# transferia/transferia

Hardware: NVIDIA H100
Metric: ChangeItems/sec on ClickBench-shaped 99-col batches (filter_rows + cast + ClickHouse native block + LZ4 frames) (higher is better)
Workload: dtype u8

## Files before the change

### transferia_b200/csrc/kernels_encode.cuh

```cuda
#pragma once
#include "device_types.cuh"

namespace tfk {

__device__ __forceinline__ uint32_t warp_incl_scan(uint32_t v) {
    const unsigned lane = threadIdx.x & 31;
#pragma unroll
    for (int d = 1; d < 32; d <<= 1) { uint32_t t = __shfl_up_sync(0xffffffffu, v, d); if (lane >= (unsigned)d) v += t; }
    return v;
}
__device__ __forceinline__ uint32_t block_excl_scan(uint32_t v, uint32_t* total, uint32_t* smem33) {
    const unsigned lane = threadIdx.x & 31, warp = threadIdx.x >> 5, nw = (blockDim.x + 31) >> 5;
    uint32_t inc = warp_incl_scan(v);
    if (lane == 31) smem33[warp] = inc;
    __syncthreads();
    if (warp == 0) {
        uint32_t w = lane < nw ? smem33[lane] : 0;
        uint32_t wi = warp_incl_scan(w);
        smem33[lane] = wi - w;
        if (lane == 31) smem33[32] = wi;
    }
    __syncthreads();
    uint32_t res = inc - v + smem33[warp];
    *total = smem33[32];
// ... 333 lines not shown
            s_size[1][threadIdx.x] = (d.nullable && n) ? n : 0;
            s_size[2][threadIdx.x] = n ? ((d.out_kind == OK_STR || d.out_kind == OK_TOSTR) ? a.col_bytes[d.str_slot] : (uint64_t)d.out_w * n) : 0;
        }
        __syncthreads();
        if (threadIdx.x == 0) {
            uint64_t p = s_run; const int m = a.ncols - base < 256 ? a.ncols - base : 256;
            for (int k = 0; k < m; k++) { s_pos[k] = p; p += s_size[0][k] + s_size[1][k] + s_size[2][k]; }
            s_run = p;
        }
        __syncthreads();
        if (c < a.ncols) {
            DCol& d = a.cols[a.out_cols[c]];
            const uint64_t p = s_pos[threadIdx.x];
            d.hdr_off = p; d.null_off = p + s_size[0][threadIdx.x]; d.out_off = d.null_off + s_size[1][threadIdx.x];
            const uint32_t hb = a.col_header_off[c], hn = (uint32_t)s_size[0][threadIdx.x];
            for (uint32_t k = 0; k < hn; k++) a.raw[p + k] = a.col_headers[hb + k];
        }
    }
    __syncthreads();
    if (threadIdx.x == 0) {
        const uint64_t p = s_run;
        a.st->raw_total = p;
        a.st->n_frames = p ? (p + a.frame_bytes - 1) / a.frame_bytes : 1;
        a.st->frame_ticket = 0;
    }
}
#endif

struct ColRegions { uint64_t values, validity, aux, offsets, heap, heap_len; };

__global__ void k_layout_columnar(LayoutArgs a, ColRegions* regions);
#ifdef TF_KERNELS_ENCODE
__global__ void __launch_bounds__(256) k_layout_columnar(LayoutArgs a, ColRegions* regions) {
    __shared__ uint64_t s_sz[5][256];
    __shared__ uint64_t s_pos[256];
    __shared__ uint64_t s_run;
    const uint64_t n = a.st->n_kept;
    if (threadIdx.x == 0) s_run = 0;
    for (int base = 0; base < a.ncols; base += 256) {
        const int k = base + threadIdx.x;
        __syncthreads();
        if (k < a.ncols) {
            const DCol& d = a.cols[a.out_cols[k]];
            const bool var = d.out_kind == OK_STR || d.out_kind == OK_MASK || d.out_kind == OK_TOSTR;
            const bool fresh = d.out_kind == OK_MASK || d.out_kind == OK_TOSTR || d.out_kind == OK_TODT;
            const uint64_t heap = (d.out_kind == OK_STR || d.out_kind == OK_TOSTR) ? a.col_bytes[d.str_slot] : (d.out_kind == OK_MASK ? 64 * n : 0);
            s_sz[0][threadIdx.x] = var ? 0 : (uint64_t)d.out_w * n;
            s_sz[1][threadIdx.x] = (d.validity && !fresh) ? (n + 7) / 8 : 0;
            s_sz[2][threadIdx.x] = (d.aux && !fresh) ? (d.type == TF_ANY ? n : 4 * n) : 0;
            s_sz[3][threadIdx.x] = var ? 4 * (n + 1) : 0;
            s_sz[4][threadIdx.x] = heap;
        }
        __syncthreads();
        if (threadIdx.x == 0) {
            uint64_t p = s_run; const int m = a.ncols - base < 256 ? a.ncols - base : 256;
            for (int q = 0; q < m; q++) { s_pos[q] = p; for (int z = 0; z < 5; z++) p += (s_sz[z][q] + 15) & ~15ull; }
            s_run = p;
        }
        __syncthreads();
        if (k < a.ncols) {
            DCol& d = a.cols[a.out_cols[k]];
            uint64_t p = s_pos[threadIdx.x]; ColRegions r;
            auto take = [&](int z) { const uint64_t at = p; p += (s_sz[z][threadIdx.x] + 15) & ~15ull; return at; };
            const uint64_t v = take(0), val = take(1), ax = take(2), of = take(3), hp = take(4);
            const bool var = d.out_kind == OK_STR || d.out_kind == OK_MASK || d.out_kind == OK_TOSTR;
            d.out_off = var ? hp : v; d.null_off = val; d.aux_off = ax; d.offs_off = of;
            r.values = var ? ~0ull : v; r.validity = s_sz[1][threadIdx.x] ? val : ~0ull; r.aux = s_sz[2][threadIdx.x] ? ax : ~0ull;
            r.offsets = var ? of : ~0ull; r.heap = var ? hp : ~0ull; r.heap_len = s_sz[4][threadIdx.x];
            regions[k] = r;
            if (var) ((uint32_t*)(a.raw + of))[n] = (uint32_t)s_sz[4][threadIdx.x];
        }
    }
    __syncthreads();
    if (threadIdx.x == 0) { a.st->raw_total = s_run; a.st->n_frames = 0; a.st->frame_ticket = 0; }
}
#endif

struct EncodeArgs {
    const DCol* cols;
    const int32_t* slots;
    const uint32_t* sel; const DState* st; uint8_t* raw;
    uint32_t* tile_sum; const uint64_t* tile_base; uint32_t ntiles_cap;
    int columnar;
};

#define TF_SLOT_NULLMAP (1 << 30)
#define TF_SLOT_AUX (1 << 29)
#define TF_SLOT_ZEROMAP (1 << 28)
#define TF_FIX_TILE_WORDS 2048
#define CH_MAX_DATE_SEC 4291747200LL

enum StreamKind { SK_COPY = 0, SK_BOOL, SK_DATE, SK_DATETIME, SK_TS64, SK_NULLMAP, SK_AUX32, SK_AUX8, SK_ZERO, SK_TODT_CH, SK_TODT_SEC };

template <int K, int INW> __device__ __forceinline__ uint64_t elem_t(const DCol& c, const uint32_t* sel, uint64_t j, uint64_t n) {
    if (j >= n) return 0;
    const uint64_t r = sel ? sel[j] : j;
    if (K == SK_ZERO) return 0;
    if (K == SK_TODT_CH || K == SK_TODT_SEC) {
        int64_t s = 0;
        if (row_valid(c, r)) s = c.type == TF_INT32 ? (int64_t)((const int32_t*)c.values)[r] : (int64_t)((const uint32_t*)c.values)[r];
        if (K == SK_TODT_SEC) return (uint64_t)s;
        if (s > CH_MAX_DATE_SEC) s = CH_MAX_DATE_SEC;
        if (s < 0) s = 0;
        return (uint64_t)s;
    }
    if (K == SK_AUX8) return (uint64_t)c.aux[r];
    if (K == SK_AUX32) return (uint64_t)((const uint32_t*)c.aux)[r];
    const bool valid = row_valid(c, r);
    if (K == SK_NULLMAP) return valid ? 0 : 1;
    if (!valid) return 0;
    if (K == SK_COPY) {
        if (INW == 1) return c.values[r];
        if (INW == 2) return ((const uint16_t*)c.values)[r];
        if (INW == 4) return ((const uint32_t*)c.values)[r];
        return ((const uint64_t*)c.values)[r];
    }
    if (K == SK_BOOL) return c.values[r] != 0;
    if (K == SK_DATE || K == SK_DATETIME) {
        int64_t s = ((const int64_t*)c.values)[r];
        const uint32_t ns = c.aux ? ((const uint32_t*)c.aux)[r] : 0;
        if (s > CH_MAX_DATE_SEC || (s == CH_MAX_DATE_SEC && ns > 0)) s = CH_MAX_DATE_SEC;
        if (s < 0) s = 0;
        return K == SK_DATE ? (uint64_t)(s / 86400) : (uint64_t)s;
    }
    const int64_t s = ((const int64_t*)c.values)[r];
    const uint32_t ns = c.aux ? ((const uint32_t*)c.aux)[r] : 0;
    return (uint64_t)(s * 1000000LL + (int64_t)(ns / 1000u));
}

template <int K, int INW, int W> __device__ __forceinline__ uint32_t stream_word_t(const DCol& c, const uint32_t* sel, uint64_t q, uint64_t n) {
    if (W == 1) return (uint32_t)elem_t<K, INW>(c, sel, 4 * q, n) | ((uint32_t)elem_t<K, INW>(c, sel, 4 * q + 1, n) << 8) |
                       ((uint32_t)elem_t<K, INW>(c, sel, 4 * q + 2, n) << 16) | ((uint32_t)elem_t<K, INW>(c, sel, 4 * q + 3, n) << 24);
    if (W == 2) return (uint32_t)(elem_t<K, INW>(c, sel, 2 * q, n) & 0xffff) | ((uint32_t)(elem_t<K, INW>(c, sel, 2 * q + 1, n) & 0xffff) << 16);
    if (W == 4) return (uint32_t)elem_t<K, INW>(c, sel, q, n);
    const uint64_t v = elem_t<K, INW>(c, sel, q >> 1, n); return (uint32_t)(v >> ((q & 1) * 32));
}

template <int K, int INW, int W> __device__ __forceinline__ void encode_stream(const DCol& c, const EncodeArgs& a, uint64_t base, uint64_t n) {
    const uint32_t m = (uint32_t)(base & 3);
    const uint64_t total = n * (uint64_t)W;
    const uint64_t T = (m + total + 3) >> 2;
    uint8_t* dst0 = a.raw + (base - m);
    const unsigned lane = threadIdx.x & 31;
    for (uint64_t t0 = (uint64_t)blockIdx.x * TF_FIX_TILE_WORDS; t0 < T; t0 += (uint64_t)gridDim.x * TF_FIX_TILE_WORDS)
#pragma unroll 2
    for (uint32_t it = 0; it < TF_FIX_TILE_WORDS / 256; it++) {
        const uint64_t t = t0 + it * 256 + threadIdx.x;
        const uint32_t wcur = (t < T) ? stream_word_t<K, INW, W>(c, a.sel, t, n) : 0;
        uint32_t wprev = __shfl_up_sync(0xffffffffu, wcur, 1);
        if (lane == 0) wprev = (m && t > 0 && t <= T) ? stream_word_t<K, INW, W>(c, a.sel, t - 1, n) : 0;
        if (t >= T) continue;
        const uint32_t val = m ? __funnelshift_r(wprev, wcur, 8 * (4 - m)) : wcur;
        const int64_t sb = (int64_t)(4 * t) - (int64_t)m;
        uint8_t* dst = dst0 + 4 * t;
        if (sb >= 0 && (uint64_t)sb + 4 <= total) *(uint32_t*)dst = val;
        else {
#pragma unroll
            for (int b = 0; b < 4; b++) { const int64_t x = sb + b; if (x >= 0 && (uint64_t)x < total) dst[b] = (uint8_t)(val >> (8 * b)); }
        }
    }
}

__global__ void k_encode_fixed(EncodeArgs a);
#ifdef TF_KERNELS_ENCODE
__global__ void __launch_bounds__(256) k_encode_fixed(EncodeArgs a) {
    const int32_t slot = a.slots[blockIdx.y];
    const DCol c = a.cols[slot & ~(TF_SLOT_NULLMAP | TF_SLOT_AUX | TF_SLOT_ZEROMAP)];
    const uint64_t n = a.st->n_kept;
    if (n == 0) return;
    const DCol& cc = c;
    if (slot & TF_SLOT_ZEROMAP) { encode_stream<SK_ZERO, 1, 1>(cc, a, c.null_off, n); return; }
    if (slot & TF_SLOT_NULLMAP) { encode_stream<SK_NULLMAP, 1, 1>(c, a, c.null_off, n); return; }
    if (slot & TF_SLOT_AUX) { if (c.type == TF_ANY) encode_stream<SK_AUX8, 1, 1>(c, a, c.aux_off, n); else encode_stream<SK_AUX32, 4, 4>(c, a, c.aux_off, n); return; }
    switch (c.out_kind) {
    case OK_COPY:
        switch (c.in_w) {
        case 1: encode_stream<SK_COPY, 1, 1>(c, a, c.out_off, n); break;
        case 2: encode_stream<SK_COPY, 2, 2>(c, a, c.out_off, n); break;
        case 4: encode_stream<SK_COPY, 4, 4>(c, a, c.out_off, n); break;
        default: encode_stream<SK_COPY, 8, 8>(c, a, c.out_off, n); break;
        }
        break;
    case OK_BOOL: encode_stream<SK_BOOL, 1, 1>(c, a, c.out_off, n); break;
    case OK_DATE: encode_stream<SK_DATE, 8, 2>(c, a, c.out_off, n); break;
    case OK_DATETIME: encode_stream<SK_DATETIME, 8, 4>(c, a, c.out_off, n); break;
    case OK_TS64: encode_stream<SK_TS64, 8, 8>(c, a, c.out_off, n); break;
    case OK_TODT: if (a.columnar) encode_stream<SK_TODT_SEC, 4, 8>(c, a, c.out_off, n); else encode_stream<SK_TODT_CH, 4, 4>(c, a, c.out_off, n); break;
    }
}
#endif

__global__ void k_pack_validity(EncodeArgs a);
#ifdef TF_KERNELS_ENCODE
__global__ void __launch_bounds__(256) k_pack_validity(EncodeArgs a) {
    const DCol c = a.cols[a.slots[blockIdx.y]];
    const uint64_t n = a.st->n_kept;
    const uint64_t b = (uint64_t)blockIdx.x * blockDim.x + threadIdx.x;
    if (b * 8 >= n) return;
    uint32_t v = 0;
#pragma unroll
    for (int k = 0; k < 8; k++) {
        const uint64_t j = b * 8 + k;
        if (j < n) { const uint64_t r = a.sel ? a.sel[j] : j; v |= (row_valid(c, r) ? 1u : 0u) << k; }
    }
    a.raw[c.null_off + b] = (uint8_t)v;
}
#endif


struct MeasureArgs { const DCol* cols; int ncols; uint64_t nrows; uint64_t* per_row; unsigned long long* total; };

__global__ void k_measure(MeasureArgs a);
#ifdef TF_KERNELS_ENCODE
__global__ void __launch_bounds__(256) k_measure(MeasureArgs a) {
    __shared__ uint32_t sm[33];
    const uint64_t r = (uint64_t)blockIdx.x * blockDim.x + threadIdx.x;
    uint64_t sz = 0;
    if (r < a.nrows) {
        sz = 24;
        for (int c = 0; c < a.ncols; c++) {
            const DCol& d = a.cols[c];
            sz += 16;
            if (!row_valid(d, r)) continue;
            switch (d.type) {
            case TF_UTF8: sz += 16 + (d.offsets[r + 1] - d.offsets[r]); break;
            case TF_ANY: sz += 16 + (d.offsets[r + 1] - d.offsets[r]); break;
            case TF_BYTES: sz += 24 + (d.offsets[r + 1] - d.offsets[r]); break;
            case TF_DATE: case TF_DATETIME: case TF_TIMESTAMP: sz += 24; break;
            default: sz += (uint64_t)d.in_w;
            }
        }
        if (a.per_row) a.per_row[r] = sz;
    }
    const uint32_t lo = (uint32_t)(sz & 0xffffffu), hi = (uint32_t)(sz >> 24);
    uint32_t tl, th; block_excl_scan(lo, &tl, sm); __syncthreads(); block_excl_scan(hi, &th, sm);
    if (threadIdx.x == 0) atomicAdd(a.total, (unsigned long long)tl + ((unsigned long long)th << 24));
}
#endif

}
```

### transferia_b200/csrc/tfgpu.cu

```cuda
#include <cuda_runtime.h>
#include <algorithm>
#include <chrono>
#include <cstdio>
#include <cstdlib>
#include <cstring>
#include <memory>
#include <string>
#include <vector>

#include "../../include/tfgpu.h"
#include "../../include/tfgpu_sink.h"
#include "plan.hpp"
#include "device_types.cuh"
#include "launch.hpp"
#include "host_internal.hpp"

using namespace tfk;

namespace {

#define CK(x) do { cudaError_t _e = (x); if (_e != cudaSuccess) throw CudaError{_e, #x}; } while (0)

inline size_t align_up(size_t v, size_t a) { return (v + a - 1) / a * a; }

// ... 203 lines not shown
    }
    pd.n_fsteps = (int)fsteps.size(); pd.n_fixed_slots = (int)pd.fixed_slots.size(); pd.n_str = (int)pd.str_slots.size(); pd.n_mask_cols = (int)pd.mask_slot_cols.size();
    pd.n_tostr = 0; for (size_t c = 0; c < pd.col_out_kind.size(); c++) if (pd.col_out_kind[c] == OK_TOSTR) pd.n_tostr++;
    std::vector<ShardCol> shcols;
    for (size_t k = 0; k < pl.shard_cols.size(); k++) shcols.push_back(ShardCol{pl.shard_cols[k], pl.shard_form[k], 0, 0});
    const std::vector<int32_t> oc(pl.out_cols.begin(), pl.out_cols.end());
    ConstImage ci;
    const size_t o_terms = ci.add(terms.data(), terms.size() * sizeof(DTerm)), o_expr_off = ci.add(expr_off.data(), expr_off.size() * 4),
                 o_fsteps = ci.add(fsteps.data(), fsteps.size() * sizeof(DFilterStep)), o_blob = ci.add(pl.blob.data(), pl.blob.size()),
                 o_hdr = ci.add(pl.col_headers.data(), pl.col_headers.size()), o_hdr_off = ci.add(pl.col_header_off.data(), pl.col_header_off.size() * 4),
                 o_fixed = ci.add(pd.fixed_slots.data(), pd.fixed_slots.size() * 4), o_str = ci.add(pd.str_slots.data(), pd.str_slots.size() * 4),
                 o_mask = ci.add(pd.mask_slot_cols.data(), pd.mask_slot_cols.size() * 4), o_keys = ci.add(keys.data(), keys.size() * sizeof(MaskKey)),
                 o_out = ci.add(oc.data(), oc.size() * 4), o_jcols = ci.add(jcols.data(), jcols.size() * sizeof(JsonCol)), o_jnames = ci.add(jnames.data(), jnames.size()),
                 o_sjcols = ci.add(sjcols.data(), sjcols.size() * sizeof(JsonCol)), o_scsv = ci.add(scsvcols.data(), scsvcols.size() * sizeof(JsonCol)),
                 o_snames = ci.add(snames.data(), snames.size()), o_shard = ci.add(shcols.data(), shcols.size() * sizeof(ShardCol));
    uint8_t* P = ci.upload(pd.consts);
    pd.d_terms = (DTerm*)(P + o_terms); pd.d_expr_off = (uint32_t*)(P + o_expr_off); pd.d_fsteps = (DFilterStep*)(P + o_fsteps); pd.d_blob = P + o_blob;
    pd.d_col_headers = P + o_hdr; pd.d_col_header_off = (uint32_t*)(P + o_hdr_off);
    pd.d_fixed_slots = (int32_t*)(P + o_fixed); pd.d_str_slots = (int32_t*)(P + o_str); pd.d_mask_slots = (int32_t*)(P + o_mask); pd.d_mask_keys = (MaskKey*)(P + o_keys);
    pd.d_out_cols = (int32_t*)(P + o_out); pd.d_jcols = (JsonCol*)(P + o_jcols); pd.d_jnames = P + o_jnames;
    pd.d_sjcols = (JsonCol*)(P + o_sjcols); pd.d_scsvcols = (JsonCol*)(P + o_scsv); pd.d_snames = P + o_snames; pd.d_shard_cols = (ShardCol*)(P + o_shard);
}

struct Sizes { uint64_t raw_bound, n_frames_max, wire_bound; uint32_t ntiles_cap, nblocks; };

Sizes compute_sizes(const tfgpu_engine* e, const PlanDev& pd, uint64_t n, const tf_col* cols, bool columnar, bool json) {
    const tfplan::Plan& pl = pd.plan;
    uint64_t raw = 64 + pl.col_headers.size();
    for (int oc : pl.out_cols) {
        const size_t c = (size_t)oc;
        if (pd.col_nullable[c]) raw += n;
        bool n2f = false; for (int q : pl.n2f_cols) if ((size_t)q == c) n2f = true;
        if (pd.col_out_kind[c] == OK_STR) raw += (n2f ? 6 : 1) * cols[c].heap_len + 5 * n;
        else if (pd.col_out_kind[c] == OK_TOSTR) raw += (in_width(cols[c].type) ? 40 * n : (n2f ? 36 : 6) * cols[c].heap_len + 8 * n) + 5 * n;
        else raw += (uint64_t)pd.col_out_w[c] * n;
        if (columnar) raw += 8 * n + 4 * (n + 1) + n / 8 + 6 * 16 + (pd.col_out_kind[c] == OK_MASK ? 64 * n : 0);
        if (json) raw += (uint64_t)(pl.in_schema[c].name.size() + 4 + 48) * n + (in_width(cols[c].type) ? 0 : (n2f ? 36 : 6) * cols[c].heap_len);
    }
    Sizes s;
    s.raw_bound = raw + 256;
    s.n_frames_max = (raw + e->frame_bytes - 1) / e->frame_bytes + 1;
    s.wire_bound = s.n_frames_max * (uint64_t)(LZ_HDR + lz4_bound(e->frame_bytes)) + 1024;
    s.ntiles_cap = (uint32_t)((n + TF_STR_TILE - 1) / TF_STR_TILE + 1);
    s.nblocks = (uint32_t)((n + 255) / 256 + 1);
    return s;
}


static void launch_offsets(tfgpu_engine* e, const uint32_t* d_len, uint64_t nrows, uint32_t nslots, uint32_t* d_off, uint64_t* d_tot, cudaStream_t s) {
    const uint32_t nchunks = (uint32_t)((nrows + CSV_OFF_CHUNK - 1) / CSV_OFF_CHUNK);
    if (!nchunks || !nslots) { TF_LAUNCH(e, k_csv_offsets, nslots ? nslots : 1, 1024, 0, s, d_len, nrows, d_off, d_tot); return; }
    e->off_scratch.ensure((size_t)nslots * nchunks * 8 + 256);
    uint64_t* cs = (uint64_t*)e->off_scratch.p;
    TF_LAUNCH(e, k_offsets_sum, dim3(nchunks, nslots), 1024, 0, s, d_len, nrows, nchunks, cs);
    TF_LAUNCH(e, k_offsets_chunks, nslots, 32, 0, s, cs, nchunks, d_tot);
    TF_LAUNCH(e, k_offsets_write, dim3(nchunks, nslots), 1024, 0, s, d_len, nrows, nchunks, cs, d_tot, d_off);
}

struct Heaps { std::vector<uint64_t> total, base; };
Heaps size_heaps(tfgpu_engine* e, const uint32_t* d_len, uint64_t nrows, uint32_t k, uint32_t* d_off, uint64_t* d_tot, uint64_t* d_base,
                 DevBuf& heap, const char* too_big) {
    cudaStream_t s = e->stream;
    launch_offsets(e, d_len, nrows, k, d_off, d_tot, s);
    Heaps h{std::vector<uint64_t>(k), std::vector<uint64_t>(k)};
    CK(cudaMemcpyAsync(h.total.data(), d_tot, (size_t)k * 8, cudaMemcpyDeviceToHost, s)); CK(cudaStreamSynchronize(s));
    uint64_t run = 0; for (uint32_t i = 0; i < k; i++) { h.base[i] = run; run += align_up(h.total[i], 16); }
    if (run >= (1ull << 32)) throw tfplan::FatalError(TF_E_FATAL_ARG, too_big);
    heap.ensure(run + 256);
    CK(cudaMemcpyAsync(d_base, h.base.data(), (size_t)k * 8, cudaMemcpyHostToDevice, s));
    return h;
}

DCol make_dcol(const tf_col& ic, int type) {
    DCol d; std::memset(&d, 0, sizeof d);
    d.type = type; d.in_w = in_width(type); d.str_slot = -1; d.mask_slot = -1;
    d.values = (const uint8_t*)ic.values; d.validity = ic.validity; d.offsets = ic.offsets; d.heap = ic.heap; d.aux = (const uint8_t*)ic.aux;
    return d;
}

void ensure_d_cols(tfgpu_engine* e, size_t nc) {
    if (e->d_cols_cap >= nc) return;
    if (e->d_cols) CK(cudaFree(e->d_cols));
    CK(cudaMalloc(&e->d_cols, sizeof(DCol) * nc)); e->d_cols_cap = nc;
}

uint32_t grid_cap(const tfgpu_engine* e, uint32_t tiles_upper, uint32_t nslots, uint32_t waves) {
    const uint32_t want = ((uint32_t)e->sm_count * 6u * waves + nslots - 1) / (nslots ? nslots : 1);
    return std::max(1u, std::min(tiles_upper, std::max(want, 8u)));
}

void run_deflate(tfgpu_engine* e, const uint8_t* text, uint64_t total, bool zlib) {
    cudaStream_t s = e->stream;
    const uint64_t nch = (total + DF_CHUNK - 1) / DF_CHUNK;
    if (nch >= (1ull << 32)) throw tfplan::FatalError(TF_E_FATAL_ARG, "row text too large to compress in one call");
    e->wire.ensure(total + nch * DF_CHUNK_OVERHEAD + 64);
    Layout L;
    const size_t o_pfx = L.take(nch * 8), o_sums = L.take(nch * 8), o_ticket = L.take(4);
    e->defl_meta.ensure(L.total());
    uint8_t* M = e->defl_meta.p;
    CK(cudaMemsetAsync(M + o_pfx, 0, nch * 8, s)); CK(cudaMemsetAsync(M + o_ticket, 0, 4, s));
    DeflateArgs da{text, total, e->wire.p, (unsigned long long*)(M + o_pfx), (uint32_t*)(M + o_sums), (uint32_t*)(M + o_ticket), (uint32_t)nch, zlib ? 1 : 0, e->d_state};
    if (nch) {
        const uint32_t grid = (uint32_t)std::min<uint64_t>(nch, (uint64_t)e->sm_count * 2);
        TF_LAUNCH(e, k_deflate_chunks, grid, DF_THREADS, df_smem().total, s, da);
    }
    TF_LAUNCH(e, k_deflate_finish, 1, 1024, 0, s, da);
}

struct ChainOut { uint8_t* errcode; uint16_t* errstep; const uint32_t* sel; bool has_sharder; };

ChainOut run_chain(tfgpu_engine* e, PlanDev& pd, uint64_t n, const tf_col* dev_cols, const uint8_t* dev_kinds, int out_fmt, const uint8_t* pre_err = nullptr, const DbzEmitArgs* dz = nullptr) {
    const bool columnar = out_fmt == 0;
    const tfplan::Plan& pl = pd.plan;
    const size_t nc = pl.in_schema.size();
    const int wire_base = out_fmt & 0xff;
    const bool dbz = wire_base == TF_WIRE_DEBEZIUM;
    const bool ser = wire_base == TF_WIRE_SER_JSON || wire_base == TF_WIRE_SER_CSV || dbz;
    const bool json_rows = wire_base == TF_WIRE_CH_JSONEACHROW || ser;
    if (ser) for (size_t c = 0; c < nc; c++) if (pd.col_out_kind[c] == OK_TOSTR && pl.in_schema[c].tf == TF_ANY)
        throw tfplan::FatalError(TF_E_FATAL_UNSUPPORTED, "serializer sinks after convert_to_string on an `any` column are not handled on the device");
    const Sizes sz = compute_sizes(e, pd, n, dev_cols, columnar, json_rows);
    cudaStream_t s = e->stream;
    if (e->tail_pending && !(out_fmt == TF_WIRE_CH_NATIVE_LZ4 && n == e->tail_nrows && (const void*)&pd == e->tail_plan && sz.n_frames_max == e->tail_nframes_max)) join_tail(e);
    const size_t nslot_alloc = (size_t)(pd.n_str > 0 ? pd.n_str : 1);
    Layout W;
    const size_t o_keep = W.take(n), o_errcode = W.take(n), o_errstep = W.take(2 * n), o_blockcnt = W.take(sz.nblocks * 4), o_blockoff = W.take(sz.nblocks * 4),
                 o_sel = W.take(n * 4), o_tile_sum = W.take(nslot_alloc * sz.ntiles_cap * 4), o_tile_base = W.take(nslot_alloc * sz.ntiles_cap * 8),
                 o_comp = W.take(sz.n_frames_max * 4), o_wire_off = W.take(sz.n_frames_max * 8), o_pfx = W.take(sz.n_frames_max * 8), o_col_bytes = W.take(nslot_alloc * 8);
    e->work.ensure(W.total());
    uint8_t* w = e->work.p;
    uint8_t* keep = w + o_keep; uint8_t* errcode = w + o_errcode; uint16_t* errstep = (uint16_t*)(w + o_errstep); uint32_t* blockcnt = (uint32_t*)(w + o_blockcnt); uint32_t* blockoff = (uint32_t*)(w + o_blockoff);
    uint32_t* tile_sum = (uint32_t*)(w + o_tile_sum); uint64_t* tile_base = (uint64_t*)(w + o_tile_base); uint64_t* col_bytes = (uint64_t*)(w + o_col_bytes);
    uint32_t* comp_size = (uint32_t*)(w + o_comp); uint64_t* wire_off = (uint64_t*)(w + o_wire_off); unsigned long long* frame_pfx = (unsigned long long*)(w + o_pfx);
    e->raw.ensure(sz.raw_bound);
    const bool lz = out_fmt == TF_WIRE_CH_NATIVE_LZ4;
    if (lz) e->wire.ensure(sz.wire_bound);
    ensure_d_cols(e, nc);
    std::vector<DCol> hc(nc); std::vector<StrictCol> strict;
    for (size_t c = 0; c < nc; c++) {
        const tf_col& ic = dev_cols[c];
        int ctype = ic.type;
        if (ic.type != pl.in_schema[c].tf) {
            const int st = ic.type, dt = pl.in_schema[c].tf;
            const bool s_num = in_width(st) && st != TF_INTERVAL && st != TF_DATE && st != TF_DATETIME && st != TF_TIMESTAMP;
            if ((st == TF_UTF8 && dt == TF_BYTES) || (st == TF_BYTES && dt == TF_UTF8)) ctype = dt;
            else if (s_num && in_width(dt) && !(st == TF_FLOAT && dt == TF_DOUBLE) && !(st == TF_BOOLEAN && dt == TF_DOUBLE)) { strict.push_back(StrictCol{(const uint8_t*)ic.values, nullptr, ic.validity, st, dt, (int32_t)c, 0}); ctype = dt; }
            else throw tfplan::FatalError(TF_E_FATAL_ARG, "column " + std::to_string(c) + ": a " + std::to_string(st) + " value cannot be strictified to the plan's column type on the device");
        }
        DCol& d = hc[c]; d = make_dcol(ic, ctype);
        d.out_kind = pd.col_out_kind[c]; d.out_w = pd.col_out_w[c];
        if (columnar && d.out_kind == OK_TODT) d.out_w = 8;
        else if (columnar && d.out_kind != OK_STR && d.out_kind != OK_MASK && d.out_kind != OK_TOSTR) { d.out_kind = OK_COPY; d.out_w = d.in_w; }
        d.nullable = pd.col_nullable[c]; d.str_slot = pd.col_str_slot[c]; d.mask_slot = pd.col_mask_slot[c];
        if (n) {
            if (d.in_w && !d.values) throw tfplan::FatalError(TF_E_FATAL_ARG, "column " + std::to_string(c) + ": values pointer is NULL");
            if (!d.in_w && !d.offsets) throw tfplan::FatalError(TF_E_FATAL_ARG, "column " + std::to_string(c) + ": offsets pointer is NULL");
        }
    }
    const uint16_t* pre_term = nullptr;
    if (!strict.empty() && n) {
        Layout S;
        const size_t o_desc = S.take(strict.size() * sizeof(StrictCol)), o_err = S.take(n), o_term = S.take(2 * n);
        std::vector<size_t> o_val(strict.size());
        for (size_t k = 0; k < strict.size(); k++) o_val[k] = S.take((size_t)in_width(strict[k].dst_tf) * n + 16);
        e->strict_stage.ensure(S.total() + 256);
        uint8_t* B = e->strict_stage.p;
        for (size_t k = 0; k < strict.size(); k++) { strict[k].dst = B + o_val[k]; hc[strict[k].col].values = B + o_val[k]; }
        CK(cudaMemcpyAsync(B + o_desc, strict.data(), strict.size() * sizeof(StrictCol), cudaMemcpyHostToDevice, s));
        if (pre_err) CK(cudaMemcpyAsync(B + o_err, pre_err, n, cudaMemcpyDeviceToDevice, s)); else CK(cudaMemsetAsync(B + o_err, 0, n, s));
        StrictArgs sa{(const StrictCol*)(B + o_desc), (int)strict.size(), n, B + o_err, (uint16_t*)(B + o_term)};
        TF_LAUNCH(e, k_strictify, (uint32_t)((n + 255) / 256), 256, 0, s, sa);
        pre_err = B + o_err; pre_term = (const uint16_t*)(B + o_term);
    }
    CK(cudaMemcpyAsync(e->d_cols, hc.data(), sizeof(DCol) * nc, cudaMemcpyHostToDevice, s));
    CK(cudaMemsetAsync(e->d_state, 0, sizeof(DState), s));
    if (!pl.n2f_cols.empty() && n) {
        const size_t k2 = pl.n2f_cols.size();
        Layout S;
        const size_t o_which = S.take(k2 * 4), o_len = S.take(k2 * n * 4), o_off = S.take(k2 * (n + 1) * 4), o_tot = S.take(k2 * 8 + 8), o_base = S.take(k2 * 8 + 8), o_err = S.take(n);
        e->n2f_stage.ensure(S.total() + 256);
        uint8_t* B = e->n2f_stage.p;
        std::vector<int32_t> which(pl.n2f_cols.begin(), pl.n2f_cols.end());
        CK(cudaMemcpyAsync(B + o_which, which.data(), k2 * 4, cudaMemcpyHostToDevice, s));
        if (pre_err) CK(cudaMemcpyAsync(B + o_err, pre_err, n, cudaMemcpyDeviceToDevice, s)); else CK(cudaMemsetAsync(B + o_err, 0, n, s));
        N2fArgs na{e->d_cols, (const int32_t*)(B + o_which), dev_kinds, n, (uint32_t*)(B + o_len), (const uint32_t*)(B + o_off), nullptr, (const uint64_t*)(B + o_base), B + o_err};
        TF_LAUNCH(e, k_n2f_sizes, dim3((uint32_t)((n + 127) / 128), (uint32_t)k2), 128, 0, s, na);
        const Heaps h = size_heaps(e, (const uint32_t*)(B + o_len), n, (uint32_t)k2, (uint32_t*)(B + o_off), (uint64_t*)(B + o_tot), (uint64_t*)(B + o_base),
                                   e->n2f_heap, "number_to_float: a rewritten column exceeds 4 GiB");
        na.heap = e->n2f_heap.p;
        TF_LAUNCH(e, k_n2f_write, dim3((uint32_t)((n + 127) / 128), (uint32_t)k2), 128, 0, s, na);
        for (size_t k = 0; k < k2; k++) { DCol& d = hc[pl.n2f_cols[k]]; d.offsets = (const uint32_t*)(B + o_off) + k * (n + 1); d.heap = e->n2f_heap.p + h.base[k]; }
        CK(cudaMemcpyAsync(e->d_cols, hc.data(), sizeof(DCol) * nc, cudaMemcpyHostToDevice, s));
        pre_err = B + o_err;
    }
    const bool sink_guard = dev_kinds && !columnar && !dbz;
    const bool has_filter = pd.n_fsteps > 0 || pre_err || sink_guard;
    e->last_wire_fmt = out_fmt;
    const uint32_t nb = (uint32_t)((n + 255) / 256);
    uint32_t* sel = (has_filter && n) ? (uint32_t*)(w + o_sel) : nullptr;
    if (sel) {
        FilterArgs fa{e->d_cols, dev_kinds, n, pd.d_fsteps, pd.n_fsteps, pd.d_expr_off, pd.d_terms, pd.d_blob, keep, errcode, errstep, blockcnt, e->d_state, pre_err, pre_term, sink_guard ? 1 : 0};
        TF_LAUNCH(e, k_filter, nb, 256, 0, s, fa);
        TF_LAUNCH(e, k_scan_blockcnt, 1, 1024, 0, s, blockcnt, blockoff, nb, e->d_state);
        TF_LAUNCH(e, k_compact_sel, nb, 256, 0, s, keep, blockoff, n, sel);
    }
    const uint32_t ntiles = (uint32_t)((n + TF_STR_TILE - 1) / TF_STR_TILE);
    const uint32_t str_gx = std::max(1u, (ntiles + TF_STR_GROUP - 1) / TF_STR_GROUP);
    EncodeArgs ea{e->d_cols, pd.d_str_slots, sel, e->d_state, e->raw.p, tile_sum, tile_base, sz.ntiles_cap, columnar ? 1 : 0};
    if (!has_filter || !n) {
        DState init; std::memset(&init, 0, sizeof init); init.n_kept = n;
        CK(cudaMemcpyAsync(e->d_state, &init, sizeof init, cudaMemcpyHostToDevice, s));
    }
    if (pl.has_sharder && n) {
        e->part_ids.ensure(n * 4 + 256);
        ShardArgs sa{e->d_cols, pd.d_shard_cols, (int)pl.shard_cols.size(), pd.d_mask_keys, sel, e->d_state, pl.shards, (uint32_t*)e->part_ids.p};
        TF_LAUNCH(e, k_shard_ids, nb, 256, 0, s, sa);
    }
    if (json_rows) {
        const uint32_t jt = (uint32_t)((n + TF_JSON_TILE - 1) / TF_JSON_TILE);
        JsonArgs ja{e->d_cols, ser ? (wire_base == TF_WIRE_SER_CSV ? pd.d_scsvcols : pd.d_sjcols) : pd.d_jcols, (int)pl.out_cols.size(), ser ? pd.d_snames : pd.d_jnames, pd.d_mask_keys, sel, e->d_state, e->raw.p,
                    (uint32_t*)e->work_json_sizes(n), tile_sum, tile_base, col_bytes,
                    dbz ? 3 : ser ? (wire_base == TF_WIRE_SER_JSON ? 1 : 2) : 0, (uint32_t)(((out_fmt & TF_WIRE_F_CLOSING_NEWLINE) ? TF_SER_NL : 0) | ((out_fmt & TF_WIRE_F_ANY_AS_STRING) ? TF_SER_AAS : 0)), errcode, errstep, DbzEmitArgs{}};
        if (dbz) { ja.jcols = pd.d_sjcols; e->dbz_keysz.ensure(n * 4 + 256); e->dbz_msgsz.ensure(n * 28 + 256); ja.dz = *dz; ja.dz.key_size = (uint32_t*)e->dbz_keysz.p; ja.dz.msg_size = (uint32_t*)e->dbz_msgsz.p; }
        if (ser && !has_filter && n) { CK(cudaMemsetAsync(errcode, 0, n, s)); CK(cudaMemsetAsync(errstep, 0, 2 * n, s)); }
        if (jt) TF_LAUNCH(e, k_json_sizes, jt, TF_JSON_TILE, 0, s, ja);
        LayoutArgs lj{e->d_cols, 0, pd.d_out_cols, pd.d_str_slots, 1, tile_sum, tile_base, sz.ntiles_cap, pd.d_col_headers, pd.d_col_header_off,
                      e->raw.p, e->d_state, n, 1, e->frame_bytes, col_bytes};
        TF_LAUNCH(e, k_layout_scan, 1, 1024, 0, s, lj);
        uint64_t json_total = 0;
        {
            CK(cudaMemcpyAsync(&json_total, col_bytes, 8, cudaMemcpyDeviceToHost, s)); CK(cudaStreamSynchronize(s));
            e->raw.ensure(json_total + 256); ja.raw = e->raw.p;
        }
        TF_LAUNCH(e, k_json_write, jt ? jt : 1, TF_JSON_TILE, 0, s, ja);
        if (ser && (out_fmt & (TF_WIRE_F_GZIP | TF_WIRE_F_ZLIB))) run_deflate(e, e->raw.p, n ? json_total : 0, (out_fmt & TF_WIRE_F_ZLIB) != 0);
        return ChainOut{errcode, errstep, sel, pl.has_sharder};
    }
    if (pd.n_str && ntiles) TF_LAUNCH(e, k_str_sizes, dim3(str_gx, pd.n_str), TF_STR_THREADS, 0, s, ea);
    LayoutArgs la{e->d_cols, (int)pl.out_cols.size(), pd.d_out_cols, pd.d_str_slots, pd.n_str, tile_sum, tile_base, sz.ntiles_cap, pd.d_col_headers, pd.d_col_header_off,
                  e->raw.p, e->d_state, n, 1, e->frame_bytes, col_bytes};
    if (pd.n_str) TF_LAUNCH(e, k_layout_scan, pd.n_str, 1024, 0, s, la);
    const int32_t* fixed_slots = pd.d_fixed_slots; uint32_t n_fixed = (uint32_t)pd.n_fixed_slots, n_valid = 0;
    if (!columnar) TF_LAUNCH(e, k_layout_finish, 1, 256, 0, s, la);
    else {
        const size_t no = pl.out_cols.size();
        if (e->d_call_cap < no) {
            if (e->d_call_slots) { CK(cudaFree(e->d_call_slots)); CK(cudaFree(e->d_regions)); }
            CK(cudaMalloc(&e->d_call_slots, sizeof(int32_t) * 3 * no)); CK(cudaMalloc(&e->d_regions, sizeof(ColRegions) * no)); e->d_call_cap = no;
        }
        std::vector<int32_t> fixed, valid;
        for (int oc : pl.out_cols) {
            const DCol& d = hc[oc];
            if (d.out_kind == OK_COPY || d.out_kind == OK_TODT) fixed.push_back(oc);
            const bool fresh = d.out_kind == OK_MASK || d.out_kind == OK_TOSTR || d.out_kind == OK_TODT;
            if (!fresh && d.aux) fixed.push_back(oc | TF_SLOT_AUX);
            if (!fresh && d.validity) valid.push_back(oc);
        }
        fixed_slots = e->d_call_slots; n_fixed = (uint32_t)fixed.size(); n_valid = (uint32_t)valid.size();
        fixed.insert(fixed.end(), valid.begin(), valid.end());
        if (!fixed.empty()) CK(cudaMemcpyAsync(e->d_call_slots, fixed.data(), fixed.size() * 4, cudaMemcpyHostToDevice, s));
        TF_LAUNCH(e, k_layout_columnar, 1, 256, 0, s, la, e->d_regions);
    }
    if (n) {
        if (n_fixed) {
            const uint32_t gx = grid_cap(e, (uint32_t)((2 * n + 2 + TF_FIX_TILE_WORDS - 1) / TF_FIX_TILE_WORDS), n_fixed, 6);
            EncodeArgs fa = ea; fa.slots = fixed_slots;
            TF_LAUNCH(e, k_encode_fixed, dim3(gx, n_fixed), 256, 0, s, fa);
        }
        if (n_valid) {
            EncodeArgs va = ea; va.slots = fixed_slots + n_fixed;
            TF_LAUNCH(e, k_pack_validity, dim3((uint32_t)((n / 8 + 256) / 256), n_valid), 256, 0, s, va);
        }
        if (pd.n_str) TF_LAUNCH(e, k_encode_str_plain, dim3(str_gx, pd.n_str), TF_STR_THREADS, 0, s, ea);
        if (pd.n_str && pd.n_tostr) TF_LAUNCH(e, k_encode_str, dim3(ntiles, pd.n_str), TF_STR_THREADS, 0, s, ea);
        if (pd.n_mask_cols) {
            MaskArgs ma{e->d_cols, pd.d_mask_slots, pd.d_mask_keys, sel, e->d_state, e->raw.p, columnar ? 1 : 0};
            TF_LAUNCH(e, k_mask_encode, dim3((uint32_t)((n + 127) / 128), pd.n_mask_cols), 128, 0, s, ma);
        }
    }
    if (lz) {
        Lz4Args za{e->raw.p, e->d_state, e->wire.p, comp_size, wire_off, frame_pfx, e->d_tail, e->frame_bytes, e->lz_phases};
        const size_t smem = lz_smem(e->frame_bytes).total;
        const uint32_t per_sm = (uint32_t)std::max<size_t>(1, std::min<size_t>(LZ_CTAS_PER_SM, (227 * 1024) / (smem + 1024)));
        const uint32_t grid = (uint32_t)std::min<uint64_t>(sz.n_frames_max, (uint64_t)e->sm_count * per_sm);
        join_tail(e);
        CK(cudaMemsetAsync(frame_pfx, 0, sz.n_frames_max * 8, s));
        TF_LAUNCH(e, k_lz4_frames, grid, LZ_THREADS, smem, s, za);
        FrameArgs fa{comp_size, wire_off, e->wire.p, e->d_tail};
        cudaStream_t s3 = e->side_stream;
        CK(cudaEventRecord(e->ev_fork, s)); CK(cudaStreamWaitEvent(s3, e->ev_fork, 0));
        TF_LAUNCH(e, k_frame_seal, (uint32_t)((sz.n_frames_max + 31) / 32), 32, SEAL_SMEM, s3, fa);
        CK(cudaEventRecord(e->ev_tail, s3));
        e->tail_pending = true; e->tail_nrows = n; e->tail_plan = (const void*)&pd; e->tail_nframes_max = sz.n_frames_max;
    }
    return ChainOut{errcode, errstep, sel, pl.has_sharder};
}

}


static bool wire_is_ser(int wire_fmt) {
    const int b = wire_fmt & 0xff;
    return (b == TF_WIRE_SER_JSON || b == TF_WIRE_SER_CSV) && (wire_fmt & ~(0xff | TF_WIRE_F_CLOSING_NEWLINE | TF_WIRE_F_ANY_AS_STRING | TF_WIRE_F_GZIP | TF_WIRE_F_ZLIB)) == 0 &&
           (wire_fmt & (TF_WIRE_F_GZIP | TF_WIRE_F_ZLIB)) != (TF_WIRE_F_GZIP | TF_WIRE_F_ZLIB);
}
static bool wire_known(int wire_fmt) { return wire_fmt == TF_WIRE_CH_NATIVE || wire_fmt == TF_WIRE_CH_NATIVE_LZ4 || wire_fmt == TF_WIRE_CH_JSONEACHROW || wire_is_ser(wire_fmt); }

static int check_batch(tfgpu_engine* e, int plan_id, const tf_batch* in, PlanDev*& pd) {
    if (!e || !in || plan_id < 0 || plan_id >= (int)e->plans.size()) return TF_E_FATAL_ARG;
    pd = e->plans[plan_id].get();
    if (in->ncols != pd->plan.in_schema.size()) return fail(e, TF_E_FATAL_ARG, "batch column count does not match the plan schema");
    if (in->nrows >= (1ull << 31)) return fail(e, TF_E_FATAL_ARG, "batch too large (>= 2^31 rows)");
    return TF_OK;
}

extern "C" {

const char* tfgpu_version(void) { return "tfgpu 0.1.0 sm_90a"; }

int tfgpu_engine_create(const char* cfg_json, const int* device_ids, int n_devices, tfgpu_engine** out) {
    if (!out) return TF_E_FATAL_ARG;
    *out = nullptr;
    int ndev = 0;
    if (cudaGetDeviceCount(&ndev) != cudaSuccess || ndev == 0) { cudaGetLastError(); return TF_E_FATAL_NODEVICE; }
    if (n_devices > 1) return TF_E_FATAL_ARG;
    auto e = std::make_unique<tfgpu_engine>();
    e->device = (n_devices == 1 && device_ids) ? device_ids[0] : 0;
    if (e->device < 0 || e->device >= ndev) return TF_E_FATAL_ARG;
    try {
        if (cfg_json && *cfg_json) {
            auto cfg = tfj::parse(cfg_json);
            double fb = cfg->get_num("frame_bytes", LZ_MAX_FRAME);
            if (fb < 1024 || fb > LZ_MAX_FRAME || ((uint32_t)fb & 15)) return TF_E_FATAL_CONFIG;
            e->frame_bytes = (uint32_t)fb;
        }
        CK(cudaSetDevice(e->device));
        cudaDeviceProp prop; CK(cudaGetDeviceProperties(&prop, e->device));
        e->sm_count = prop.multiProcessorCount;
        CK(cudaStreamCreateWithFlags(&e->own_stream, cudaStreamNonBlocking));
        e->stream = e->own_stream;
        CK(cudaStreamCreateWithFlags(&e->side_stream, cudaStreamNonBlocking));
        CK(cudaEventCreateWithFlags(&e->ev_tail, cudaEventDisableTiming));
        CK(cudaMalloc(&e->d_tail, 64)); CK(cudaMemset(e->d_tail, 0, 64));
        CK(cudaEventCreateWithFlags(&e->ev_fork, cudaEventDisableTiming));
        CK(cudaMalloc(&e->d_state, sizeof(DState)));
        const struct { const void* k; size_t smem; } big_smem[] = {
            {(const void*)k_lz4_frames, lz_smem(LZ_MAX_FRAME).total}, {(const void*)k_frame_seal, SEAL_SMEM},
            {(const void*)k_dbz_pass1, DBZ_STAGE}, {(const void*)k_deflate_chunks, df_smem().total}};
        for (const auto& b : big_smem) CK(cudaFuncSetAttribute(b.k, cudaFuncAttributeMaxDynamicSharedMemorySize, (int)b.smem));
    } catch (const CudaError& c) { return c.e == cudaErrorMemoryAllocation ? TF_E_RETRY_OOM : TF_E_RETRY_LAUNCH; }
// ... 1036 lines not shown
```

Before: 1.147 billion.

## Rewrite fixed-width column encode as source-row tiles with shared-memory compaction

Replaces the output-word gather encoder, which read each kept row through the sel index, with a source-row-tiled kernel. Each thread loads 8 consecutive input rows with vector loads, compacts the kept rows into shared memory using the keep flags, per-256-row block offsets and a warp scan, then the block writes the output region with aligned 16-byte stores via funnel shifts. The aim is to turn scattered gathers and unaligned byte handling into coalesced reads and wide writes. In exchange it uses 16KB of shared memory per CTA, adds two syncthreads per tile, fixes launch bounds at 6 CTAs, and reads all rows, including filtered ones.

```diff
diff --git a/transferia_b200/csrc/kernels_encode.cuh b/transferia_b200/csrc/kernels_encode.cuh
--- a/transferia_b200/csrc/kernels_encode.cuh
+++ b/transferia_b200/csrc/kernels_encode.cuh
@@ -439,110 +439,157 @@
     const uint32_t* sel; const DState* st; uint8_t* raw;
     uint32_t* tile_sum; const uint64_t* tile_base; uint32_t ntiles_cap;
     int columnar;
+    const uint8_t* keep; const uint32_t* blockoff; uint64_t nrows;
 };
 
 #define TF_SLOT_NULLMAP (1 << 30)
 #define TF_SLOT_AUX (1 << 29)
 #define TF_SLOT_ZEROMAP (1 << 28)
-#define TF_FIX_TILE_WORDS 2048
+#define TF_FIX_ROWS 8
+#define TF_FIX_TILE (256 * TF_FIX_ROWS)
+#define TF_FIX_TILES_PER_CTA 4
 #define CH_MAX_DATE_SEC 4291747200LL
 
 enum StreamKind { SK_COPY = 0, SK_BOOL, SK_DATE, SK_DATETIME, SK_TS64, SK_NULLMAP, SK_AUX32, SK_AUX8, SK_ZERO, SK_TODT_CH, SK_TODT_SEC };
 
-template <int K, int INW> __device__ __forceinline__ uint64_t elem_t(const DCol& c, const uint32_t* sel, uint64_t j, uint64_t n) {
-    if (j >= n) return 0;
-    const uint64_t r = sel ? sel[j] : j;
+template <int K> __device__ __forceinline__ uint64_t cast_elem(const DCol& c, uint64_t v, uint64_t ns, bool valid) {
     if (K == SK_ZERO) return 0;
     if (K == SK_TODT_CH || K == SK_TODT_SEC) {
         int64_t s = 0;
-        if (row_valid(c, r)) s = c.type == TF_INT32 ? (int64_t)((const int32_t*)c.values)[r] : (int64_t)((const uint32_t*)c.values)[r];
+        if (valid) s = c.type == TF_INT32 ? (int64_t)(int32_t)(uint32_t)v : (int64_t)(uint32_t)v;
         if (K == SK_TODT_SEC) return (uint64_t)s;
         if (s > CH_MAX_DATE_SEC) s = CH_MAX_DATE_SEC;
         if (s < 0) s = 0;
         return (uint64_t)s;
     }
-    if (K == SK_AUX8) return (uint64_t)c.aux[r];
-    if (K == SK_AUX32) return (uint64_t)((const uint32_t*)c.aux)[r];
-    const bool valid = row_valid(c, r);
+    if (K == SK_AUX8 || K == SK_AUX32) return v;
     if (K == SK_NULLMAP) return valid ? 0 : 1;
     if (!valid) return 0;
-    if (K == SK_COPY) {
-        if (INW == 1) return c.values[r];
-        if (INW == 2) return ((const uint16_t*)c.values)[r];
-        if (INW == 4) return ((const uint32_t*)c.values)[r];
-        return ((const uint64_t*)c.values)[r];
-    }
-    if (K == SK_BOOL) return c.values[r] != 0;
+    if (K == SK_COPY) return v;
+    if (K == SK_BOOL) return v != 0;
     if (K == SK_DATE || K == SK_DATETIME) {
-        int64_t s = ((const int64_t*)c.values)[r];
-        const uint32_t ns = c.aux ? ((const uint32_t*)c.aux)[r] : 0;
+        int64_t s = (int64_t)v;
         if (s > CH_MAX_DATE_SEC || (s == CH_MAX_DATE_SEC && ns > 0)) s = CH_MAX_DATE_SEC;
         if (s < 0) s = 0;
         return K == SK_DATE ? (uint64_t)(s / 86400) : (uint64_t)s;
     }
-    const int64_t s = ((const int64_t*)c.values)[r];
-    const uint32_t ns = c.aux ? ((const uint32_t*)c.aux)[r] : 0;
-    return (uint64_t)(s * 1000000LL + (int64_t)(ns / 1000u));
-}
-
-template <int K, int INW, int W> __device__ __forceinline__ uint32_t stream_word_t(const DCol& c, const uint32_t* sel, uint64_t q, uint64_t n) {
-    if (W == 1) return (uint32_t)elem_t<K, INW>(c, sel, 4 * q, n) | ((uint32_t)elem_t<K, INW>(c, sel, 4 * q + 1, n) << 8) |
-                       ((uint32_t)elem_t<K, INW>(c, sel, 4 * q + 2, n) << 16) | ((uint32_t)elem_t<K, INW>(c, sel, 4 * q + 3, n) << 24);
-    if (W == 2) return (uint32_t)(elem_t<K, INW>(c, sel, 2 * q, n) & 0xffff) | ((uint32_t)(elem_t<K, INW>(c, sel, 2 * q + 1, n) & 0xffff) << 16);
-    if (W == 4) return (uint32_t)elem_t<K, INW>(c, sel, q, n);
-    const uint64_t v = elem_t<K, INW>(c, sel, q >> 1, n); return (uint32_t)(v >> ((q & 1) * 32));
-}
-
-template <int K, int INW, int W> __device__ __forceinline__ void encode_stream(const DCol& c, const EncodeArgs& a, uint64_t base, uint64_t n) {
-    const uint32_t m = (uint32_t)(base & 3);
-    const uint64_t total = n * (uint64_t)W;
-    const uint64_t T = (m + total + 3) >> 2;
-    uint8_t* dst0 = a.raw + (base - m);
-    const unsigned lane = threadIdx.x & 31;
-    for (uint64_t t0 = (uint64_t)blockIdx.x * TF_FIX_TILE_WORDS; t0 < T; t0 += (uint64_t)gridDim.x * TF_FIX_TILE_WORDS)
-#pragma unroll 2
-    for (uint32_t it = 0; it < TF_FIX_TILE_WORDS / 256; it++) {
-        const uint64_t t = t0 + it * 256 + threadIdx.x;
-        const uint32_t wcur = (t < T) ? stream_word_t<K, INW, W>(c, a.sel, t, n) : 0;
-        uint32_t wprev = __shfl_up_sync(0xffffffffu, wcur, 1);
-        if (lane == 0) wprev = (m && t > 0 && t <= T) ? stream_word_t<K, INW, W>(c, a.sel, t - 1, n) : 0;
-        if (t >= T) continue;
-        const uint32_t val = m ? __funnelshift_r(wprev, wcur, 8 * (4 - m)) : wcur;
-        const int64_t sb = (int64_t)(4 * t) - (int64_t)m;
-        uint8_t* dst = dst0 + 4 * t;
-        if (sb >= 0 && (uint64_t)sb + 4 <= total) *(uint32_t*)dst = val;
-        else {
-#pragma unroll
-            for (int b = 0; b < 4; b++) { const int64_t x = sb + b; if (x >= 0 && (uint64_t)x < total) dst[b] = (uint8_t)(val >> (8 * b)); }
-        }
+    return (uint64_t)((int64_t)v * 1000000LL + (int64_t)(ns / 1000u));
+}
+
+template <int B> __device__ __forceinline__ void load_rows(const uint8_t* p, uint64_t r0, int nr, uint64_t (&v)[TF_FIX_ROWS]) {
+    const uint8_t* q = p + r0 * B;
+    if (nr == TF_FIX_ROWS && ((uintptr_t)q & (B == 1 ? 7 : 15)) == 0) {
+        if (B == 1) {
+            const uint64_t x = *(const uint64_t*)q;
+#pragma unroll
+            for (int k = 0; k < 8; k++) v[k] = (x >> (8 * k)) & 0xff;
+        } else {
+            uint32_t w[2 * B];
+#pragma unroll
+            for (int i = 0; i < B / 2; i++) { const uint4 x = ((const uint4*)q)[i]; w[4 * i] = x.x; w[4 * i + 1] = x.y; w[4 * i + 2] = x.z; w[4 * i + 3] = x.w; }
+#pragma unroll
+            for (int k = 0; k < 8; k++) {
+                if (B == 2) v[k] = (w[k >> 1] >> (16 * (k & 1))) & 0xffff;
+                else if (B == 4) v[k] = w[k];
+                else v[k] = (uint64_t)w[2 * k] | ((uint64_t)w[2 * k + 1] << 32);
+            }
+        }
+        return;
+    }
+#pragma unroll
+    for (int k = 0; k < 8; k++) {
+        const uint64_t r = r0 + k;
+        v[k] = k >= nr ? 0 : B == 1 ? p[r] : B == 2 ? ((const uint16_t*)p)[r] : B == 4 ? ((const uint32_t*)p)[r] : ((const uint64_t*)p)[r];
+    }
+}
+
+__device__ __forceinline__ uint4 bytes_at(const uint4 a, const uint4 b, uint32_t d) {
+    uint32_t x0 = a.x, x1 = a.y, x2 = a.z, x3 = a.w, x4 = b.x, x5 = b.y;
+    if (d & 8) { x0 = x2; x1 = x3; x2 = x4; x3 = x5; x4 = b.z; x5 = b.w; }
+    if (d & 4) { x0 = x1; x1 = x2; x2 = x3; x3 = x4; x4 = x5; }
+    const uint32_t sh = 8 * (d & 3);
+    return make_uint4(__funnelshift_r(x0, x1, sh), __funnelshift_r(x1, x2, sh), __funnelshift_r(x2, x3, sh), __funnelshift_r(x3, x4, sh));
+}
+
+template <int K, int INW, int W> __device__ __forceinline__ void encode_tile(const DCol& c, const EncodeArgs& a, uint64_t base, uint8_t* stage) {
+    constexpr bool VALUES = K != SK_ZERO && K != SK_NULLMAP;
+    constexpr bool VALIDITY = K != SK_ZERO && K != SK_AUX8 && K != SK_AUX32;
+    constexpr bool NANOS = K == SK_DATE || K == SK_DATETIME || K == SK_TS64;
+    const unsigned warp = threadIdx.x >> 5;
+    const uint64_t n = a.nrows, ntiles = (n + TF_FIX_TILE - 1) / TF_FIX_TILE;
+    for (uint64_t tile = blockIdx.x; tile < ntiles; tile += gridDim.x) {
+        const uint64_t t0 = tile * TF_FIX_TILE, r0 = t0 + (uint64_t)threadIdx.x * TF_FIX_ROWS;
+        const int nr = r0 < n ? (int)min((uint64_t)TF_FIX_ROWS, n - r0) : 0;
+        const uint32_t b0 = (uint32_t)(t0 / 256), nb = (uint32_t)((n + 255) / 256);
+        uint64_t kf = 0, j0, j1, bbase;
+        if (a.keep) {
+            if (nr == TF_FIX_ROWS) kf = *(const uint64_t*)(a.keep + r0);
+            else for (int k = 0; k < nr; k++) kf |= (uint64_t)a.keep[r0 + k] << (8 * k);
+            j0 = a.blockoff[b0];
+            j1 = b0 + 8 < nb ? a.blockoff[b0 + 8] : a.st->n_kept;
+            bbase = b0 + warp < nb ? a.blockoff[b0 + warp] : j1;
+        } else {
+            j0 = t0; j1 = min(n, t0 + TF_FIX_TILE); bbase = t0 + 256 * warp;
+        }
+        uint64_t v[TF_FIX_ROWS], ns[TF_FIX_ROWS];
+        if (VALUES) load_rows<INW>(K == SK_AUX8 || K == SK_AUX32 ? c.aux : c.values, r0, nr, v);
+#pragma unroll
+        for (int k = 0; k < TF_FIX_ROWS; k++) ns[k] = 0;
+        if (NANOS && c.aux) load_rows<4>(c.aux, r0, nr, ns);
+        const uint32_t vb = (VALIDITY && c.validity && nr) ? c.validity[r0 >> 3] : 0xffu;
+        if (j1 == j0) continue;
+        uint32_t km = 0;
+#pragma unroll
+        for (int k = 0; k < TF_FIX_ROWS; k++) km |= (a.keep ? ((kf >> (8 * k)) & 0xff) != 0 : k < nr) ? 1u << k : 0u;
+        const uint32_t cnt = __popc(km);
+        uint32_t j = (uint32_t)(bbase - j0) + warp_incl_scan(cnt) - cnt;
+#pragma unroll
+        for (int k = 0; k < TF_FIX_ROWS; k++) {
+            if (!((km >> k) & 1)) continue;
+            const uint64_t x = cast_elem<K>(c, VALUES ? v[k] : 0, ns[k], (vb >> k) & 1);
+            if (W == 1) stage[j] = (uint8_t)x;
+            else if (W == 2) ((uint16_t*)stage)[j] = (uint16_t)x;
+            else if (W == 4) ((uint32_t*)stage)[j] = (uint32_t)x;
+            else ((uint64_t*)stage)[j] = x;
+            j++;
+        }
+        __syncthreads();
+        const uint64_t ob = base + W * j0, oe = base + W * j1;
+        const uint64_t lo = min((uint64_t)((ob + 15) & ~15ull), oe), hi = max((uint64_t)(oe & ~15ull), lo);
+        if (threadIdx.x < 16) { const uint64_t x = ob + threadIdx.x; if (x < lo) a.raw[x] = stage[x - ob]; }
+        else if (threadIdx.x < 32) { const uint64_t x = hi + threadIdx.x - 16; if (x < oe) a.raw[x] = stage[x - ob]; }
+        const uint32_t d = (uint32_t)(lo - ob) & 15;
+        for (uint64_t g = lo + 16 * threadIdx.x; g < hi; g += 16 * blockDim.x) {
+            const uint32_t s0 = (uint32_t)(g - ob) & ~15u;
+            *(uint4*)(a.raw + g) = bytes_at(*(const uint4*)(stage + s0), *(const uint4*)(stage + s0 + 16), d);
+        }
+        __syncthreads();
     }
 }
 
 __global__ void k_encode_fixed(EncodeArgs a);
 #ifdef TF_KERNELS_ENCODE
-__global__ void __launch_bounds__(256) k_encode_fixed(EncodeArgs a) {
+__global__ void __launch_bounds__(256, 6) k_encode_fixed(EncodeArgs a) {
+    __shared__ __align__(16) uint8_t stage[TF_FIX_TILE * 8 + 16];
     const int32_t slot = a.slots[blockIdx.y];
     const DCol c = a.cols[slot & ~(TF_SLOT_NULLMAP | TF_SLOT_AUX | TF_SLOT_ZEROMAP)];
-    const uint64_t n = a.st->n_kept;
-    if (n == 0) return;
-    const DCol& cc = c;
-    if (slot & TF_SLOT_ZEROMAP) { encode_stream<SK_ZERO, 1, 1>(cc, a, c.null_off, n); return; }
-    if (slot & TF_SLOT_NULLMAP) { encode_stream<SK_NULLMAP, 1, 1>(c, a, c.null_off, n); return; }
-    if (slot & TF_SLOT_AUX) { if (c.type == TF_ANY) encode_stream<SK_AUX8, 1, 1>(c, a, c.aux_off, n); else encode_stream<SK_AUX32, 4, 4>(c, a, c.aux_off, n); return; }
+    if (slot & TF_SLOT_ZEROMAP) { encode_tile<SK_ZERO, 1, 1>(c, a, c.null_off, stage); return; }
+    if (slot & TF_SLOT_NULLMAP) { encode_tile<SK_NULLMAP, 1, 1>(c, a, c.null_off, stage); return; }
+    if (slot & TF_SLOT_AUX) { if (c.type == TF_ANY) encode_tile<SK_AUX8, 1, 1>(c, a, c.aux_off, stage); else encode_tile<SK_AUX32, 4, 4>(c, a, c.aux_off, stage); return; }
     switch (c.out_kind) {
     case OK_COPY:
         switch (c.in_w) {
-        case 1: encode_stream<SK_COPY, 1, 1>(c, a, c.out_off, n); break;
-        case 2: encode_stream<SK_COPY, 2, 2>(c, a, c.out_off, n); break;
-        case 4: encode_stream<SK_COPY, 4, 4>(c, a, c.out_off, n); break;
-        default: encode_stream<SK_COPY, 8, 8>(c, a, c.out_off, n); break;
-        }
-        break;
-    case OK_BOOL: encode_stream<SK_BOOL, 1, 1>(c, a, c.out_off, n); break;
-    case OK_DATE: encode_stream<SK_DATE, 8, 2>(c, a, c.out_off, n); break;
-    case OK_DATETIME: encode_stream<SK_DATETIME, 8, 4>(c, a, c.out_off, n); break;
-    case OK_TS64: encode_stream<SK_TS64, 8, 8>(c, a, c.out_off, n); break;
-    case OK_TODT: if (a.columnar) encode_stream<SK_TODT_SEC, 4, 8>(c, a, c.out_off, n); else encode_stream<SK_TODT_CH, 4, 4>(c, a, c.out_off, n); break;
+        case 1: encode_tile<SK_COPY, 1, 1>(c, a, c.out_off, stage); break;
+        case 2: encode_tile<SK_COPY, 2, 2>(c, a, c.out_off, stage); break;
+        case 4: encode_tile<SK_COPY, 4, 4>(c, a, c.out_off, stage); break;
+        default: encode_tile<SK_COPY, 8, 8>(c, a, c.out_off, stage); break;
+        }
+        break;
+    case OK_BOOL: encode_tile<SK_BOOL, 1, 1>(c, a, c.out_off, stage); break;
+    case OK_DATE: encode_tile<SK_DATE, 8, 2>(c, a, c.out_off, stage); break;
+    case OK_DATETIME: encode_tile<SK_DATETIME, 8, 4>(c, a, c.out_off, stage); break;
+    case OK_TS64: encode_tile<SK_TS64, 8, 8>(c, a, c.out_off, stage); break;
+    case OK_TODT: if (a.columnar) encode_tile<SK_TODT_SEC, 4, 8>(c, a, c.out_off, stage); else encode_tile<SK_TODT_CH, 4, 4>(c, a, c.out_off, stage); break;
     }
 }
 #endif
diff --git a/transferia_b200/csrc/tfgpu.cu b/transferia_b200/csrc/tfgpu.cu
--- a/transferia_b200/csrc/tfgpu.cu
+++ b/transferia_b200/csrc/tfgpu.cu
@@ -309,11 +309,6 @@
     if (e->d_cols_cap >= nc) return;
     if (e->d_cols) CK(cudaFree(e->d_cols));
     CK(cudaMalloc(&e->d_cols, sizeof(DCol) * nc)); e->d_cols_cap = nc;
-}
-
-uint32_t grid_cap(const tfgpu_engine* e, uint32_t tiles_upper, uint32_t nslots, uint32_t waves) {
-    const uint32_t want = ((uint32_t)e->sm_count * 6u * waves + nslots - 1) / (nslots ? nslots : 1);
-    return std::max(1u, std::min(tiles_upper, std::max(want, 8u)));
 }
 
 void run_deflate(tfgpu_engine* e, const uint8_t* text, uint64_t total, bool zlib) {
@@ -433,7 +428,7 @@
     }
     const uint32_t ntiles = (uint32_t)((n + TF_STR_TILE - 1) / TF_STR_TILE);
     const uint32_t str_gx = std::max(1u, (ntiles + TF_STR_GROUP - 1) / TF_STR_GROUP);
-    EncodeArgs ea{e->d_cols, pd.d_str_slots, sel, e->d_state, e->raw.p, tile_sum, tile_base, sz.ntiles_cap, columnar ? 1 : 0};
+    EncodeArgs ea{e->d_cols, pd.d_str_slots, sel, e->d_state, e->raw.p, tile_sum, tile_base, sz.ntiles_cap, columnar ? 1 : 0, sel ? keep : nullptr, sel ? blockoff : nullptr, n};
     if (!has_filter || !n) {
         DState init; std::memset(&init, 0, sizeof init); init.n_kept = n;
         CK(cudaMemcpyAsync(e->d_state, &init, sizeof init, cudaMemcpyHostToDevice, s));
@@ -490,9 +485,8 @@
     }
     if (n) {
         if (n_fixed) {
-            const uint32_t gx = grid_cap(e, (uint32_t)((2 * n + 2 + TF_FIX_TILE_WORDS - 1) / TF_FIX_TILE_WORDS), n_fixed, 6);
             EncodeArgs fa = ea; fa.slots = fixed_slots;
-            TF_LAUNCH(e, k_encode_fixed, dim3(gx, n_fixed), 256, 0, s, fa);
+            TF_LAUNCH(e, k_encode_fixed, dim3((uint32_t)((n + (uint64_t)TF_FIX_TILE * TF_FIX_TILES_PER_CTA - 1) / ((uint64_t)TF_FIX_TILE * TF_FIX_TILES_PER_CTA)), n_fixed), 256, 0, s, fa);
         }
         if (n_valid) {
             EncodeArgs va = ea; va.slots = fixed_slots + n_fixed;
```

After: 1.163 billion (median of 6 runs). About the same (+1.4%).
